# zhuker/lamejs

Measured on AMD Instinct MI355X. Metric: 1152-sample frames/s encoded (44.1kHz 128kbps CBR); bit-exact, higher is better.
Workload: dtype f64; 1 GPU; BASELINE configs[2]: stereo 44.1kHz 128kbps CBR, 1 stream(s) x 100000 synthetic sine frames per GPU; input=Int16 PCM resident in HBM, output=MP3 bytes in HBM, seed_repaired_frames=0, distinct_streams=1, distinct_devices=1

## Files before the change

### lamejs_amd/csrc/k_quant.h

```cpp
#pragma once
#include "lhip_defs.h"
#include "lhip_wave.h"
#include "lhip_math.h"
#include "lhip_layout.h"

namespace lhip {

struct GI {
    double xrpow_max;
    int part2_3_length, big_values, count1, global_gain, scalefac_compress, block_type;
    int table_select[3], subblock_gain[4];
    int region0_count, region1_count, preflag, scalefac_scale, count1table_select;
    int part2_length, sfb_lmax, sfb_smin, psy_lmax, sfbmax, psymax, sfbdivide;
    int count1bits, max_nonzero_coeff;
    int firstcut;
    int tail0;
};

struct NoiseRes { double max_noise; int over_count, over_SSD, bits; };

LHIP_DEV void uni_gi(GI& g) {
    g.xrpow_max = unid(g.xrpow_max);
    g.part2_3_length = uni(g.part2_3_length); g.big_values = uni(g.big_values); g.count1 = uni(g.count1); g.global_gain = uni(g.global_gain);
    g.scalefac_compress = uni(g.scalefac_compress); g.block_type = uni(g.block_type);
    for (int i = 0; i < 3; i++) g.table_select[i] = uni(g.table_select[i]);
    for (int i = 0; i < 4; i++) g.subblock_gain[i] = uni(g.subblock_gain[i]);
    g.region0_count = uni(g.region0_count); g.region1_count = uni(g.region1_count); g.preflag = uni(g.preflag); g.scalefac_scale = uni(g.scalefac_scale);
    g.count1table_select = uni(g.count1table_select); g.part2_length = uni(g.part2_length); g.sfb_lmax = uni(g.sfb_lmax); g.sfb_smin = uni(g.sfb_smin);
    g.psy_lmax = uni(g.psy_lmax); g.sfbmax = uni(g.sfbmax); g.psymax = uni(g.psymax); g.sfbdivide = uni(g.sfbdivide);
    g.count1bits = uni(g.count1bits); g.max_nonzero_coeff = uni(g.max_nonzero_coeff); g.firstcut = uni(g.firstcut); g.tail0 = uni(g.tail0);
}

#if defined(LHIP_PHASE_PROF) && !defined(LHIP_HOSTSIM)
#define PH_BEGIN() const unsigned long long ph_t0_ = __builtin_amdgcn_s_memtime()
#define PH_END(L, id) do { if (lane == 0) { (L).prof[id] += (unsigned int)(__builtin_amdgcn_s_memtime() - ph_t0_); (L).prof[32 + id] += 1; } } while (0)
#define PH_MARK(L, id, t) do { const unsigned long long n_ = __builtin_amdgcn_s_memtime(); if (lane == 0) { (L).prof[id] += (unsigned int)(n_ - (t)); (L).prof[32 + id] += 1; } (t) = n_; } while (0)
#define PH_NOW() __builtin_amdgcn_s_memtime()
#else
#define PH_BEGIN() do {} while (0)
#define PH_END(L, id) do {} while (0)
#define PH_MARK(L, id, t) do {} while (0)
#define PH_NOW() 0ull
#endif
#ifdef LHIP_PROF_BALANCE
#define PH_MARKB(L, id, t) PH_MARK(L, id, t)
#else
#define PH_MARKB(L, id, t) do {} while (0)
#endif
enum { PH_INIT, PH_XRPOW, PH_XMIN, PH_QUANTIZE, PH_COUNT, PH_NOISE, PH_BALANCE, PH_SFSTORE, PH_HUFFDIV, PH_PUBLISH, PH_COPY, PH_TOTAL,
       PH_C_LOAD, PH_C_QUADS, PH_C_MAX, PH_C_SUMS, PH_C_FIN, PH_N_WALK, PH_N_TERMS, PH_N_SUMS, PH_Q_MASK, PH_Q_LINES, PH_N, PH_DRAIN = 29 ,
       PH_N_LINES = 30, PH_N_FOLD = 31 ,
       PH_B_TRIG = 22, PH_B_AMP = 23, PH_B_BREAK = 24, PH_B_BITCOUNT = 25  };

enum { QT_N = 256 };
enum { HL_T1 = 0, HL_T2 = 4, HL_T3 = 13, HL_T5 = 22, HL_T6 = 38, HL_T7 = 54, HL_T8 = 90, HL_T9 = 126, HL_T10 = 162, HL_T11 = 226,
       HL_T12 = 290, HL_T13 = 354, HL_T14 = 610, HL_T15 = 866, HL_EHI = 1122, HL_ELO = 1378, HL_END = 1634 };
LHIP_DEV int hl_off(int t) {
    switch (t) {
        case 1: return HL_T1; case 2: return HL_T2; case 3: return HL_T3; case 5: return HL_T5; case 6: return HL_T6;
        case 7: return HL_T7; case 8: return HL_T8; case 9: return HL_T9; case 10: return HL_T10; case 11: return HL_T11;
        case 12: return HL_T12; case 13: return HL_T13; case 14: return HL_T14; case 15: return HL_T15; default: return 0;
    }
}
struct alignas(16) QuantTabs {
    float pow43[QT_N], adj43[QT_N];
    float ipow20[Q_MAX], pow20[Q_MAX + Q_MAX2 + 1];
    int32_t sfb_l[SBMAX_l + 1], sfb_s[SBMAX_s + 1], pretab[SBMAX_l];
    uint16_t hoff[16];
    uint8_t hlen[HL_END];
    uint8_t t32l[16], t33l[16];
    uint8_t l2s_long[576], l2s_short[576];
    uint32_t bvtab[289];
    uint8_t huf_tbl_noESC[16], ht_xlen[34];
    uint16_t ht_linmax[34];
    struct PlanEnt { uint32_t d0, d1, pw; } plan[30];
    uint32_t sbc[16];
    uint32_t fold_marks[2][64];
    uint16_t wpre_long[24], wpre_short[40];
    int16_t psfb21[PSFB21 + 1], psfb12[PSFB12 + 1];
    float ath_psfb[PSFB21 + PSFB12], fact_psfb[2];
};

LHIP_DEV void q_fill_plans(QuantTabs& Q, int tid, int nthr);

LHIP_DEV void q_load_tabs(const Tables& T, QuantTabs& Q, int tid, int nthr) {
    q_fill_plans(Q, tid, nthr);
    for (int i = tid; i < QT_N; i += nthr) { Q.pow43[i] = T.pow43[i]; Q.adj43[i] = T.adj43[i]; }
    for (int i = tid; i < Q_MAX; i += nthr) Q.ipow20[i] = T.ipow20[i];
    for (int i = tid; i < Q_MAX + Q_MAX2 + 1; i += nthr) Q.pow20[i] = T.pow20[i];
    for (int i = tid; i < 16; i += nthr) { Q.t32l[i] = (uint8_t)T.t32l[i]; Q.t33l[i] = (uint8_t)T.t33l[i]; }
    for (int i = tid; i < SBMAX_l + 1; i += nthr) Q.sfb_l[i] = T.sfb_l[i];
    for (int i = tid; i < SBMAX_s + 1; i += nthr) Q.sfb_s[i] = T.sfb_s[i];
    for (int i = tid; i < SBMAX_l; i += nthr) Q.pretab[i] = T.pretab[i];
    for (int i = tid; i < 16; i += nthr)
        Q.sbc[i] = (uint32_t)T.slen1_n[i] | ((uint32_t)T.slen2_n[i] << 8) | ((uint32_t)T.scale_long[i] << 16) | ((uint32_t)T.scale_short[i] << 24);
    for (int i = tid; i < 289; i += nthr) Q.bvtab[i] = (uint32_t)T.bvtab[i];
    for (int i = tid; i < 15; i += nthr) Q.huf_tbl_noESC[i] = (uint8_t)T.huf_tbl_noESC[i];
    for (int i = tid; i < 34; i += nthr) { Q.ht_xlen[i] = (uint8_t)T.ht_xlen[i]; Q.ht_linmax[i] = (uint16_t)T.ht_linmax[i]; }
    if (tid == 0) { Q.hoff[0] = 0; Q.hoff[4] = 0; }
    for (int t = 1; t < 16; t++) {
        if (t == 4) continue;
        const int xl = T.ht_xlen[t];
        const int n = (t == 14) ? 256 : xl * xl, off = hl_off(t);
        if (tid == 0) Q.hoff[t] = (uint16_t)off;
        for (int i = tid; i < n; i += nthr) Q.hlen[off + i] = (uint8_t)T.ht_hlen[T.ht_off[t] + i];
    }
    for (int i = tid; i < 256; i += nthr) { Q.hlen[HL_EHI + i] = (uint8_t)(T.largetbl[i] >> 16); Q.hlen[HL_ELO + i] = (uint8_t)(T.largetbl[i] & 0xffff); }
    for (int d = tid; d < 576; d += nthr) {
        int sfb = 0;
        while (T.sfb_l[sfb + 1] <= d) sfb++;
        Q.l2s_long[d] = (uint8_t)sfb;
        sfb = 0;
        while (3 * T.sfb_s[sfb + 1] <= d) sfb++;
        const int st = T.sfb_s[sfb], w = T.sfb_s[sfb + 1] - st;
        const int r = d - 3 * st, win = r / w, l = st + (r - win * w);
        Q.l2s_short[d] = (uint8_t)(3 * sfb + win);
        (void)l;
    }
    for (int e = tid; e < PSFB21 + 1; e += nthr) Q.psfb21[e] = (int16_t)T.psfb21[e];
    for (int e = tid; e < PSFB12 + 1; e += nthr) Q.psfb12[e] = (int16_t)T.psfb12[e];
    for (int e = tid; e < PSFB21 + PSFB12; e += nthr) Q.ath_psfb[e] = e < PSFB21 ? T.ATH_psfb21[e] : T.ATH_psfb12[e - PSFB21];
    if (tid == 0) { Q.fact_psfb[0] = T.longfact[21]; Q.fact_psfb[1] = T.shortfact[12]; }
    for (int e = tid; e < 2 * 64; e += nthr) Q.fold_marks[e >> 6][e & 63] = (uint32_t)T.fold_marks[e];
    for (int e = tid; e < 24; e += nthr) Q.wpre_long[e] = (uint16_t)T.wpre[e];
    for (int e = tid; e < 40; e += nthr) Q.wpre_short[e] = (uint16_t)T.wpre[24 + e];
}

LHIP_DEV void q_copy_tabs(const Tables& T, QuantTabs& Q, int tid, int nthr) {
    static_assert(sizeof(QuantTabs) % 16 == 0, "QuantTabs is copied in 16-byte pieces");
    struct alignas(16) V4 { uint32_t a, b, c, d; };
    const V4* src = (const V4*)T.qtabs_img;
    V4* dst = (V4*)&Q;
    for (int i = tid; i < (int)(sizeof(QuantTabs) / 16); i += nthr) dst[i] = src[i];
}

struct QuantLds {
    float xr[576];
    union {
        float xrpow[576];
        struct { int32_t bstat[16][SBMAX_l + 2]; int16_t cand[21][16]; } hd;
    };
    int16_t ixw[576];
    int32_t sfw[SFBMAX + 1], sfb[SFBMAX + 1];
    int16_t width[SFBMAX + 1], window[SFBMAX + 1], start[SFBMAX + 2];
    float xmin[SFBMAX + 1], distort[SFBMAX + 1];
    double rxmin[SFBMAX + 1];
    int32_t pn_step[SFBMAX + 1];
    float pn_dist[SFBMAX + 1];
    union {
        double pn_x[SFBMAX + 1];
        int16_t hmax[5][24];
    };
    int16_t pn_cls[SFBMAX + 1];
    int32_t qmode[SFBMAX + 1];
    float bstep[SFBMAX + 1];
    int8_t sf_gr0[2][SFBMAX + 1];
    union {
        struct { int32_t r01_bits[24], r01_div[24], r0_tbl[24], r1_tbl[24], r2_bits[24], r2_tbl[24]; };
        double nsum[SFBMAX + 1];
        struct { int32_t bs_tab[BS_TAB_MAX], bs_asg[BS_TAB_MAX]; } memo;
    };
    alignas(8) uint32_t rdesc[4][2];
    int32_t gkeep[24];
    double ath_pseudo[PSFB21 + PSFB12];
#ifdef LHIP_PHASE_PROF
    unsigned int prof[64];
#endif
};

LHIP_DEV double ipow20(const QuantTabs& Q, int x) { return (double)Q.ipow20[x]; }
LHIP_DEV double pow20(const QuantTabs& Q, int x) { return (double)Q.pow20[x + Q_MAX2]; }
LHIP_DEV double pow43v(const Tables& T, const QuantTabs& Q, int i) {
    float v = Q.pow43[i < QT_N ? i : QT_N - 1];
    if (i >= QT_N) v = T.pow43[i];
    return (double)v;
}
// ... 702 lines not shown
        if (q.kind == 0) { b = 0; t = 0; }
        if (q.kind == 6) { b = 0; t = 63; }
        PV_(r) = t | ((q.kind == 6) << 6) | (b << 8);
    }
#if LHIP_NL == 1
    const int pv0 = pv[0], pv1_ = pv[1], pv2 = pv[2];
#else
    const int pv0 = wave_bcast(pv1, 0), pv1_ = wave_bcast(pv1, 1), pv2 = wave_bcast(pv1, 2);
#endif
#define APPLY(PV, SLOT) do { const int t_ = (PV) & 63; if ((PV) & 64) bits = LARGE_BITS; else bits += (PV) >> 8; g.table_select[SLOT] = (t_ == 63) ? -1 : t_; } while (0)
    if (use2) APPLY(pv2, 2);
    if (0 < a1) APPLY(pv0, 0);
    if (a1 < a2) APPLY(pv1_, 1);
#undef APPLY
#undef LP_
#undef PV_
    if (use_prev && g.block_type == NORM_TYPE) *pn_sfb_count1 = cnt1_norm;
    PH_MARK(L, PH_C_FIN, tm_);
    return bits;
}

struct PrevNoise { int gain, sfb_count1; };

template <int NR>
LHIP_DEV int q_count_bits(const Tables& T, GI& g, const int32_t* scalefac, int16_t* ix, int use_pn, PrevNoise& pn, int* asg, int lane, QuantLds& L, const QuantTabs& Q) {
    *asg = 0;
    {
        const double ip = ipow20(Q, g.global_gain);
        if (g.xrpow_max * ip > (double)IXMAX_VAL * (1.0 - 0x1p-50)) {
            const double w = (double)IXMAX_VAL / ip;
            if (g.xrpow_max > w) return LARGE_BITS;
        }
    }
    int vx[NR], vy[NR];
    { PH_BEGIN(); q_quantize<NR>(T, g, scalefac, ix, use_pn, use_pn ? pn.gain : 0, use_pn ? pn.sfb_count1 : 0, vx, vy, lane, L, Q); PH_END(L, PH_QUANTIZE); }
    int cnt1 = pn.sfb_count1;
    PH_BEGIN();
    int amask = 0;
    const int r = q_noquant_count_bits<NR>(T, g, ix, vx, vy, use_pn, &cnt1, &amask, lane, L, Q);
    *asg = pack_cond_fields(g, amask);
    if (use_pn) pn.sfb_count1 = cnt1;
    PH_END(L, PH_COUNT);
    return r;
}
template <int SKIP>
LHIP_DEV int q_count_bits_rounds(const Tables& T, GI& g, const int32_t* scalefac, int16_t* ix, int use_pn, PrevNoise& pn, int* asg, int lane, QuantLds& L, const QuantTabs& Q) {
    if constexpr (SKIP != 0) {
        if (g.tail0) { LHIP_ROUND_COUNT(head); return q_count_bits<NPL_HEAD>(T, g, scalefac, ix, use_pn, pn, asg, lane, L, Q); }
    }
    LHIP_ROUND_COUNT(full);
    return q_count_bits<NPL>(T, g, scalefac, ix, use_pn, pn, asg, lane, L, Q);
}

struct NoiseCommit { int fresh, step, cls; float dist; double x; };
LHIP_DEV void q_noise_commit(const GI& g, const NoiseCommit& nc, PrevNoise& pn, int lane, QuantLds& L) {
    lane = fresh_lane(lane);
    LHIP_LANE_ONCE(sfb, 0, g.psymax) {
        if (nc.fresh) { L.pn_step[sfb] = nc.step; L.pn_dist[sfb] = nc.dist; L.pn_x[sfb] = nc.x; L.pn_cls[sfb] = (int16_t)nc.cls; }
    }
    pn.gain = g.global_gain;
    wave_sync();
}
LHIP_DEV void q_calc_noise_(const Tables& T, const GI& g, const int32_t* scalefac, const int16_t* ix, NoiseRes* res,
                           int use_pn, PrevNoise& pn, int need_max, int lane, QuantLds& L, const QuantTabs& Q, NoiseCommit* defer = nullptr) {
    lane = fresh_lane(lane);
    unsigned long long tm_ = PH_NOW(); (void)tm_;
    const int is_short = g.block_type == SHORT_TYPE;
    const int may_big = !(g.xrpow_max * ipow20(Q, g.global_gain) < (double)(QT_N - 1));
#if LHIP_NL == 1
    const uint8_t* l2s = line2sfb(Q, g.block_type);
    int over = 0, ssd = 0;
    uint64_t m_fresh = 0;
    (void)may_big; (void)is_short;
    for (int sfb = 0; sfb < g.psymax; sfb++) {
        const int s = sf_step(Q, g, scalefac, L.window, sfb);
        if (!(use_pn && L.pn_step[sfb] == s)) m_fresh |= 1ull << sfb;
        L.qmode[sfb] = s;
        L.bstep[sfb] = Q.pow20[s + Q_MAX2];
    }
    PH_MARK(L, PH_N_WALK, tm_);
    {
        double sacc = 0.0;
        for (int j = 0; j < 576; j++) {
            const int bnd = l2s[j];
            if (j == 0 || l2s[j - 1] != bnd) sacc = 0.0;
            const double x = __builtin_fma(-pow43v(T, Q, ix[j]), (double)L.bstep[bnd < SFBMAX + 1 ? bnd : SFBMAX], d_abs((double)L.xr[j]));
            sacc += x * x;
            if (j == 575 || l2s[j + 1] != bnd) L.nsum[bnd] = sacc;
        }
    }
    PH_MARK(L, PH_N_FOLD, tm_);
    for (int sfb = 0; sfb < g.psymax; sfb++) {
        int cls;
        if (!((m_fresh >> sfb) & 1)) { L.distort[sfb] = L.pn_dist[sfb]; cls = L.pn_cls[sfb]; }
        else {
            const double noise = L.nsum[sfb], b = (double)L.xmin[sfb], rb = L.rxmin[sfb];
            const double x = rb != 0.0 ? div_by_f32(noise, b, rb) : noise / b;
            L.distort[sfb] = (float)x;
            if (use_pn) { L.pn_step[sfb] = L.qmode[sfb]; const double nf = (double)(float)noise; L.pn_dist[sfb] = (float)(rb != 0.0 ? div_by_f32(nf, b, rb) : nf / b); }
            cls = need_max ? -1 : noise_class(x);
            int cls_cache = cls;
            if (cls < 0) {
                const double l = v8_log10_pos(x > 1E-20 ? x : 1E-20);
                cls = noise_class_of_log(l); cls_cache = noise_class_of_log((double)(float)l);
            }
            if (use_pn) { L.pn_x[sfb] = x; L.pn_cls[sfb] = (int16_t)cls_cache; }
            else L.nsum[sfb] = x;
        }
        if (cls > 0) { ssd += cls * cls; over++; }
    }
    PH_MARK(L, PH_N_TERMS, tm_);
    if (use_pn) pn.gain = g.global_gain;
    res->over_count = over; res->over_SSD = ssd;
    res->max_noise = 0.0;
    if (need_max || over == 0) {
        double max_noise = -20.0;
        for (int sfb = 0; sfb < g.psymax; sfb++) {
            const bool fresh = (m_fresh >> sfb) & 1;
            const double x = (fresh && !use_pn) ? L.nsum[sfb] : L.pn_x[sfb];
            const double l = v8_log10_pos(x > 1E-20 ? x : 1E-20);
            const double nl = fresh ? l : (double)(float)l;
            if (nl > max_noise) max_noise = nl;
        }
        res->max_noise = max_noise;
    }
#else
    int my_step = 0, my_fresh = 0;
    LHIP_LANE_ONCE(sfb, 0, g.psymax) {
        my_step = sf_step(Q, g, scalefac, L.window, sfb);
        my_fresh = !(use_pn && L.pn_step[sfb] == my_step);
        L.bstep[sfb] = Q.pow20[my_step + Q_MAX2];
    }
    const uint64_t m_fresh = wave_ballot(my_fresh);
    const int hib = m_fresh ? 63 - (int)__builtin_clzll(m_fresh) : 0;
    const int maxlen = m_fresh ? (int)(is_short ? Q.wpre_short[hib] : Q.wpre_long[hib]) : 0;
    wave_sync();
    PH_MARK(L, PH_N_WALK, tm_);
    enum { NLN = 576 / LHIP_NL };
    static_assert(NLN == 9, "QuantTabs::fold_marks is laid out for 9 lines per lane");
    {
        double tq[NLN], keep[NLN];
        int lastb[NLN];
        const uint32_t marks = Q.fold_marks[is_short][lane];
        const uint8_t* l2s = line2sfb(Q, g.block_type);
#define NOISE_TERMS(IDX) _Pragma("unroll") for (int k = 0; k < NLN; k++) { \
            const int j = NLN * lane + k; \
            const int bnd = l2s[j]; \
            const float bstep = L.bstep[bnd]; \
            const float xa = L.xr[j]; const int iv = ix[j]; \
            const float pw = Q.pow43[IDX]; \
            const double x = __builtin_fma(-(double)pw, (double)bstep, d_abs((double)xa)); \
            tq[k] = x * x; \
            keep[k] = one_unless_bit(marks, k); \
            lastb[k] = bnd; \
        }
        if (!may_big) { NOISE_TERMS(iv) } else { NOISE_TERMS(iv < QT_N ? iv : QT_N - 1) }
#undef NOISE_TERMS
        if (may_big) {
#pragma unroll
            for (int k = 0; k < NLN; k++) {
                const int j = NLN * lane + k;
                const int iv = ix[j];
                if (iv >= QT_N) {
                    const double x = __builtin_fma(-(double)T.pow43[iv], (double)L.bstep[lastb[k]], d_abs((double)L.xr[j]));
                    tq[k] = x * x;
                }
            }
        }
        PH_MARK(L, PH_N_LINES, tm_);
        const int nsteps = (maxlen + NLN - 1) / NLN + 1;
        double carry = 0.0;
        for (int st = 0; st + 1 < nsteps; st++) {
            double sacc = carry;
#pragma unroll
            for (int k = 0; k < NLN; k++) sacc = __builtin_fma(sacc, keep[k], tq[k]);
            carry = wave_shr1d(sacc, 0.0);
        }
        {
            double sacc = carry;
#pragma unroll
            for (int k = 0; k < NLN; k++) { sacc = __builtin_fma(sacc, keep[k], tq[k]); tq[k] = sacc; }
        }
#pragma unroll
        for (int k = 0; k < NLN; k++) if ((marks >> (16 + k)) & 1u) L.nsum[lastb[k]] = tq[k];
        wave_sync();
        PH_MARK(L, PH_N_FOLD, tm_);
    }
    double x = 1.0;
    int cls = 0;
    const int fresh = my_fresh;
    LHIP_LANE_ONCE(sfb, 0, g.psymax) {
        if (!fresh) {
            L.distort[sfb] = L.pn_dist[sfb];
            x = L.pn_x[sfb];
            cls = L.pn_cls[sfb];
        } else {
            const double noise = L.nsum[sfb], b = (double)L.xmin[sfb], rb = L.rxmin[sfb];
            const double nf = (double)(float)noise;
            x = div_by_f32(noise, b, rb);
            double xf = div_by_f32(nf, b, rb);
            if (rb == 0.0) { x = noise / b; xf = nf / b; }
            L.distort[sfb] = (float)x;
            if (defer) { defer->step = my_step; defer->dist = (float)xf; }
            else if (use_pn) { L.pn_step[sfb] = my_step; L.pn_dist[sfb] = (float)xf; }
            cls = need_max ? -1 : noise_class(x);
        }
    }
    PH_MARK(L, PH_N_TERMS, tm_);
    int cls_cache = cls;
    int have_log = 0;
    double nl = -20.0;
    if (wave_any(cls < 0)) {
        LHIP_LANE_ONCE(sfb, 0, g.psymax) {
            const double l = v8_log10_pos(x > 1E-20 ? x : 1E-20);
            const double lf = (double)(float)l;
            nl = fresh ? l : lf;
            if (fresh) { cls = noise_class_of_log(l); cls_cache = noise_class_of_log(lf); }
        }
        have_log = 1;
    }
    int over = 0, ssd = 0;
    if (defer) { defer->fresh = 0; LHIP_LANE_ONCE(sfb, 0, g.psymax) { defer->fresh = use_pn && fresh; defer->x = x; defer->cls = cls_cache; } }
    LHIP_LANE_ONCE(sfb, 0, g.psymax) {
        if (!defer && use_pn && fresh) { L.pn_x[sfb] = x; L.pn_cls[sfb] = (int16_t)cls_cache; }
        if (cls > 0) { ssd = cls * cls; over = 1; }
    }
    if (use_pn && !defer) pn.gain = g.global_gain;
    {
        const int os = wave_sum((ssd << 6) | over);
        res->over_count = os & 63; res->over_SSD = os >> 6;
    }
    res->max_noise = 0.0;
    if (need_max || res->over_count == 0) {
        double max_noise = -20.0;
        if (!have_log) {
            LHIP_LANE_ONCE(sfb, 0, g.psymax) {
                const double l = v8_log10_pos(x > 1E-20 ? x : 1E-20);
                nl = fresh ? l : (double)(float)l;
            }
        }
// ... 1496 lines not shown
```

### lamejs_amd/csrc/lhip_api.cpp

```cpp
#include "../../include/lamejs_hip.h"
#include "lhip_defs.h"
#include "lhip_wave.h"
#include "lhip_math.h"
#include "lhip_layout.h"
#include "k_psy.h"
#include "k_fb.h"
#include "k_quant.h"
#if !defined(LHIP_HOSTSIM) || defined(LHIP_WAVESIM)
#include "k_quant_tail.h"
#endif
#include "k_quant_fast.h"
#include "k_bits.h"
#include "k_crc.h"
#include "k_ingest.h"
#include "k_gain.h"

#include <string>
#include <vector>
#include <map>
#include <mutex>
#include <thread>
#include <atomic>
#include <memory>
#include <cstring>
// ... 564 lines not shown
    (void)device;
#endif
    return 0;
}

int lhip_set_hip_stream(int device, void* hip_stream) {
#ifndef LHIP_HOSTSIM
    if (device < 0) { if (hipGetDevice(&device) != hipSuccess) return LHIP_ERR_INTERNAL; }
#else
    if (device < 0) device = 0;
#endif
    Context* ctx = get_context(device);
    std::lock_guard<std::mutex> lk(ctx->mu);
    ctx->stream = hip_stream;
    return 0;
}

void lhip_last_batch_stats(int64_t* frames, int64_t* repaired_frames, int64_t* repair_iterations) {
#ifndef LHIP_HOSTSIM
    if (g_stat_pending) {
        Context* ctx = g_stat_pending;
        g_stat_pending = nullptr;
        std::lock_guard<std::mutex> lk(ctx->mu);
        int32_t fx[3] = {0, 0, 0};
        WorkSet& ws = ctx->ws;
        void* st = ctx->stream;
        if (rt::set_device(ctx->device) && rt::d2h(fx, (const int32_t*)ws.nflagged.p + FX_STATS, sizeof fx, st) && rt::sync(st)) {
            g_stat_repaired = fx[0]; g_stat_iters = fx[1];
            if (fx[2]) set_err("seed-chain repair did not converge");
        }
    }
#endif
    if (frames) *frames = g_stat_frames;
    if (repaired_frames) *repaired_frames = g_stat_repaired;
    if (repair_iterations) *repair_iterations = g_stat_iters;
}

int lhip_debug_last_paths(uint32_t* mask) {
    if (!mask) { set_err("lhip_debug_last_paths: null argument"); return LHIP_ERR_INTERNAL; }
    *mask = g_last_paths;
    return 0;
}

int64_t lhip_debug_read(int what, void* dst, size_t cap) {
    if (what == 11) {
        if (!dst) { set_err("lhip_debug_read: null argument"); return LHIP_ERR_INTERNAL; }
        const size_t n = cap < sizeof g_last_quant ? cap : sizeof g_last_quant; memcpy(dst, &g_last_quant, n); return (int64_t)n;
    }
#ifdef LHIP_HOSTSIM
    if (what == 10) {
        const int64_t v[2] = {(int64_t)__atomic_load_n(&round_stats().head, __ATOMIC_RELAXED), (int64_t)__atomic_load_n(&round_stats().full, __ATOMIC_RELAXED)};
        const size_t n = cap < sizeof v ? cap : sizeof v; memcpy(dst, v, n); return (int64_t)n;
    }
#endif
#ifdef LHIP_PHASE_PROF
    if (what == 9) { const size_t n = cap < sizeof g_call_prof ? cap : sizeof g_call_prof; memcpy(dst, g_call_prof, n); return (int64_t)n; }
#endif
    Context* ctx = nullptr;
    { std::lock_guard<std::mutex> lk(g_ctx_mu); for (auto& kv : g_ctx) if (kv.second->ws.have_last) ctx = kv.second.get(); }
    if (!ctx) { set_err("no batch has run"); return LHIP_ERR_INTERNAL; }
    std::lock_guard<std::mutex> lk(ctx->mu);
    rt::set_device(ctx->device);
    const WorkSet& ws = ctx->ws;
    const Workspace& W = ws.lastW;
    const size_t GC = (size_t)W.ngslots * ws.lastC;
    const void* src = nullptr; size_t n = 0;
    switch (what) {
        case 0: src = W.xr; n = GC * 576 * 4; break;
        case 1: src = W.blocktype; n = GC * 4; break;
        case 2: src = W.E; n = (size_t)W.ngslots * ws.lastCp * E_STRIDE * 4; break;
        case 3: src = W.ath_adjust; n = (size_t)W.nfslots * 8; break;
        case 4: src = W.side; n = (size_t)W.nframes_total * 2 * ws.lastC * sizeof(GrSide); break;
        case 5: src = W.sb; n = GC * SB_STRIDE * 4; break;
        case 6: src = W.peaks; n = GC * PK_STRIDE * 4; break;
        case 7: src = W.prof; n = PROF_BYTES; break;
        case 8: src = W.nflagged; n = 256; break;
        default: set_err("unknown tap"); return LHIP_ERR_INTERNAL;
    }
    if (n > cap) n = cap;
    if (!rt::d2h(dst, src, n, ctx->stream) || !rt::sync(ctx->stream)) return LHIP_ERR_INTERNAL;
    return (int64_t)n;
}

int lhip_stream_info(const lhip_stream* s, lhip_stream_info_t* info) {
    if (!s || s->magic != 0x4c484950) { set_err("bad stream handle"); return LHIP_ERR_BAD_HANDLE; }
    if (!info) { set_err("lhip_stream_info: null argument"); return LHIP_ERR_INTERNAL; }
    if (!s->tag) { set_err("lhip_stream_info: the stream was not created with the infoTag option (its totals are not kept)"); return LHIP_ERR_INTERNAL; }
    const TagTotals& v = *s->tag;
    info->frames = v.frames; info->audio_bytes = v.bytes; info->music_crc = v.crc & 0xffff; info->delay = s->ts->tag.delay;
    info->padding = v.padding < 0 ? -1 : (int32_t)v.padding; info->tag_bytes = s->ts->tag.size;
    return 0;
}
int64_t lhip_info_tag(lhip_stream* s, uint8_t* out, size_t cap) {
    if (!s || s->magic != 0x4c484950) { set_err("bad stream handle"); return LHIP_ERR_BAD_HANDLE; }
    if (!s->tag) { set_err("lhip_info_tag: the stream was not created with the infoTag option"); return LHIP_ERR_INTERNAL; }
    if (s->tag->moved) { set_err("lhip_info_tag: the stream was moved with lhip_seek or lhip_state_set; state blobs do not carry the tag's totals (combining the tags of shards is not supported)"); return LHIP_ERR_INTERNAL; }
    if (!s->tag->flushed) { set_err("lhip_info_tag: the stream has not been flushed (the tag reports the totals and the end padding of the complete stream)"); return LHIP_ERR_INTERNAL; }
    const size_t n = (size_t)s->ts->tag.size;
    if (!out || cap < n) { set_err("output buffer too small"); return LHIP_ERR_BUFFER_TOO_SMALL; }
    uint32_t radio = 0;
    if (s->gain) {
        int32_t tenth = 0; int64_t windows = 0, samples = 0;
        const int rc = lhip_replay_gain(s, &tenth, &windows, &samples);
        if (rc < 0) return rc;
        if (rc == 0) radio = gain_tag_field(tenth);
    }
// ... 234 lines not shown
```

### lamejs_amd/csrc/lhip_defs.h

```cpp
#pragma once
#include <stdint.h>
#include <stddef.h>

#ifdef LHIP_HOSTSIM
#include <math.h>
#include <string.h>
#include <stdio.h>
#include <stdlib.h>
#define LHIP_DEV static inline
#ifdef LHIP_WAVESIM
#define LHIP_NL 64
#else
#define LHIP_NL 1
#endif
#else
#include <hip/hip_runtime.h>
#define LHIP_DEV static __device__ __forceinline__
#define LHIP_NL 64
#endif

#ifdef LHIP_HOSTSIM
typedef const double* lhip_ctab;
#define LHIP_CTAB(p) (p)
#define LHIP_SCHED_FENCE() ((void)0)
// ... 15 lines not shown

namespace lhip {

enum {
    SBMAX_l = 22, SBMAX_s = 13, SBPSY_l = 21, SBPSY_s = 12, PSFB21 = 6, PSFB12 = 6,
    CBANDS = 64, BLKSIZE = 1024, HBLKSIZE = 513, BLKSIZE_s = 256, HBLKSIZE_s = 129, SFBMAX = 39,
    NORM_TYPE = 0, START_TYPE = 1, SHORT_TYPE = 2, STOP_TYPE = 3,
    IXMAX_VAL = 8206, PRECALC_SIZE = IXMAX_VAL + 2, Q_MAX = 257, Q_MAX2 = 116, LARGE_BITS = 100000,
    MAX_BITS_PER_CHANNEL = 4095, MAX_BITS_PER_GRANULE = 7680,
    FRAME = 1152, GRAN = 576, MF_NEEDED = 1904, MF_INIT = 528
};

#define LHIP_SQRT2 1.41421356237309504880

struct Tables {
    int channels_out, mode, mode_gr, version, samplerate_index, bitrate_index, brate, out_samplerate,
        sideinfo_len, frac_SpF, noise_shaping, noise_shaping_amp, noise_shaping_stop, subblock_gain,
        use_best_huffman, full_outer_loop, substep_shaping, sfb21_extra, quant_comp, quant_comp_short,
        short_blocks_coupled, useTemporal, ATH_useAdjust, athaa_loudapprox, copyright, original, emphasis,
        extension, error_protection, npart_l, npart_s, n_version_bytes,
        n_s3_ll,
       
        in_samplerate, rs_filter_l, rs_bpc,
        rs_ratio,
        rs_frac,
        psy_channels,
        disable_reservoir;
    double scale, attackthre, attackthre_s, interChRatio, masking_lower_long, masking_lower_short,
        ATH_aaSensitivityP, ATH_floor, decay, ma_max_i1, ma_max_i2, ma_max_m, VO_SCALE, resample_ratio,
        msfix, ATHlower;
    const float *rs_blackfilt;
    const float *amp_filter, *ATH_l, *ATH_s, *ATH_psfb21, *ATH_psfb12, *ATH_cb_l, *ATH_cb_s, *eql_w,
        *pow43, *adj43, *ipow20, *pow20, *longfact, *shortfact, *rnumlines_l, *bo_l_weight, *bo_s_weight,
        *s3_ll, *s3_ss, *window, *window_s, *mld_l, *mld_s;
    const int32_t *sfb_l, *sfb_s, *psfb21, *psfb12, *bv_scf, *numlines_l, *numlines_s, *bo_l, *bm_l, *bo_s,
        *bm_s, *s3ind, *s3ind_s, *fft_rv_tbl, *mdct_order, *pretab, *scfsi_band, *slen1_n, *slen2_n,
        *slen1_tab, *slen2_tab, *scale_short, *scale_long, *huf_tbl_noESC, *version_bytes, *ht_xlen,
        *ht_linmax, *ht_off, *ht_code, *ht_hlen, *largetbl, *table23, *table56, *t32l, *t33l;
    const double *fht_twiddle, *fht_costab, *enwindow, *mdct_win, *ma_tab, *ma_table1, *ma_table2, *ma_table3,
        *hpf_fircoef;
    const int32_t *s3off_l, *s3off_s;
    const int32_t *lineoff_l, *lineoff_s;
    const double *amp_by_out;
    int amp_mask;
    const int32_t *psy_fold; int psy_maxlen_l;
    const int32_t *bvtab;
    const void *qtabs_img;
    const int32_t *fold_marks, *wpre;
    double scale_left, scale_right;
    int channels_in,
        do_scale, do_scale_left, do_scale_right,
        in_mix;
    float pcm_limit;
};

enum { BS_TAB_MAX = 24 };
struct GrSide {
    int32_t part2_3_length, part2_length, big_values, count1, global_gain, scalefac_compress, block_type;
    int32_t table_select[3], subblock_gain[3];
    int32_t region0_count, region1_count, preflag, scalefac_scale, count1table_select;
    int32_t sfbmax, sfbdivide;
    int32_t active;
    int32_t bs_start, bs_step_in, bs_gain;
    int32_t targ_bits;
    int32_t scfsi;
    int32_t scalefac[SFBMAX];
    int32_t bs_ntab, bs_tab[BS_TAB_MAX];
    int32_t bs_asg[BS_TAB_MAX], bs_state;
    int32_t mode_ext;
};

}
```

### lamejs_amd/csrc/lhip_kernels.h

```cpp
#pragma once
#define XCD_GRID(n) (8 * (((n) + 7) / 8))
static __device__ __forceinline__ int xcd_item(int b, int n) { const int it = (b & 7) * ((n + 7) >> 3) + (b >> 3); return it < n && (b >> 3) < ((n + 7) >> 3) ? it : -1; }
__global__ __launch_bounds__(64) void g_load(Tables T, Workspace W, const StreamDesc* SD, const StreamIO* IO) { kb_load(T, W, SD, IO, blockIdx.x, threadIdx.x); }
__global__ __launch_bounds__(64) void g_save(Tables T, Workspace W, const StreamDesc* SD, const StreamIO* IO) { kb_save(T, W, SD, IO, blockIdx.x, threadIdx.x); }
#ifndef LHIP_WPB
#define LHIP_WPB 4
#endif
enum { WPB = LHIP_WPB };
#define XCD_GRID_W(n) XCD_GRID(((n) + WPB - 1) / WPB)
static __device__ __forceinline__ int xcd_wave_item(int n, int* lane) {
    const int wv = __builtin_amdgcn_readfirstlane((int)(threadIdx.x >> 6));
    *lane = (int)(threadIdx.x & 63);
    const int g = xcd_item(blockIdx.x, (n + WPB - 1) / WPB);
    const int it = g * WPB + wv;
    return (g >= 0 && it < n) ? it : -1;
}
#define WAVE_LDS(TYPE, NAME) __shared__ TYPE NAME##_[WPB]; TYPE& NAME = NAME##_[__builtin_amdgcn_readfirstlane((int)(threadIdx.x >> 6))]
__global__ __launch_bounds__(64 * WPB) void g_psyA(Tables T, Workspace W, const StreamDesc* SD, const StreamIO* IO, int chn0, int nch) {
    WAVE_LDS(PsyALds, L);
    int lane;
    const int it = xcd_wave_item(W.ngslots * nch, &lane);
    if (it >= 0) kb_psyA(T, W, SD, IO, it / nch, chn0 + it % nch, lane, L);
}
__global__ __launch_bounds__(256) void g_prep(Tables T, Workspace W, const StreamDesc* SD, const StreamIO* IO, int nstreams) {
// ... 46 lines not shown
    __shared__ QuantTabs Q;
    __shared__ QuantLds L[QWAVES];
    __shared__ TailShare TS;
#ifndef LHIP_PHASE_PROF
    static_assert(QWAVES * sizeof(QuantLds) + sizeof(QuantTabs) + sizeof(TailShare) <= 80 * 1024, "g_quant: LDS budget for 2 workgroups per CU exceeded");
#endif
    const QArgs* A = (const QArgs*)__builtin_amdgcn_kernarg_segment_ptr();
    q_copy_tabs(A->T, Q, threadIdx.x, 64 * QWAVES);
    if (threadIdx.x == 0) TS.drawing = QWAVES;
    if (threadIdx.x < QWAVES) TS.offer[threadIdx.x].state = 0;
    const bool tail_help_on = !RESV && A->T.channels_out == 2;
    __syncthreads();
    const int wv = __builtin_amdgcn_readfirstlane(threadIdx.x >> 6);
#ifdef LHIP_PHASE_PROF
    L[wv].prof[threadIdx.x & 63] = 0;
#endif
#if defined(LHIP_PHASE_PROF) || defined(LHIP_WAVE_TIMES)
    const unsigned long long wave_t0_ = wall_clock64();
#endif
    int hint[3] = {-1, -1, -1};
    for (;;) {
        const int fslot = next_frame_slot(A->W.work_ctr + A->ctr);
        if (fslot >= A->nfs) break;
        if constexpr (!RESV) kb_quant_th<SKIP>(A->T, A->pb, A->W, A->SD, fslot, threadIdx.x & 63, L[wv], Q, hint, TS, wv);
        else kb_quant<0, RESV, SKIP>(A->T, A->pb, A->W, A->SD, fslot, A->chain, threadIdx.x & 63, L[wv], Q, -1, nullptr, nullptr, nullptr);
        hint[0] = __builtin_amdgcn_readfirstlane(hint[0]); hint[1] = __builtin_amdgcn_readfirstlane(hint[1]); hint[2] = __builtin_amdgcn_readfirstlane(hint[2]);
    }
    if (tail_help_on) tail_help<SKIP>(A->T, A->pb, A->W, A->SD, threadIdx.x & 63, L, wv, QWAVES, Q, TS);
#ifdef LHIP_PHASE_PROF
    atomicAdd((unsigned long long*)A->W.prof + (threadIdx.x & 63), (unsigned long long)L[wv].prof[threadIdx.x & 63]);
#endif
#if defined(LHIP_PHASE_PROF) || defined(LHIP_WAVE_TIMES)
    {
        const int wid = blockIdx.x * QWAVES + wv;
        if ((threadIdx.x & 63) == 0 && wid < 8192) { A->W.prof[64 + 2 * wid] = wave_t0_; A->W.prof[64 + 2 * wid + 1] = wall_clock64(); }
    }
#endif
}
template <int RESV, int SKIP> __global__ __launch_bounds__(128, LHIP_QOCC) void g_quant_pair(QArgs a_unused) {
    __shared__ QuantTabs Q;
    __shared__ QuantLds L[2];
    __shared__ int mbox[4];
    const QArgs* A = (const QArgs*)__builtin_amdgcn_kernarg_segment_ptr();
    q_copy_tabs(A->T, Q, threadIdx.x, 128);
    __syncthreads();
    const int wv = __builtin_amdgcn_readfirstlane(threadIdx.x >> 6);
    kb_quant<1, RESV, SKIP>(A->T, A->pb, A->W, A->SD, blockIdx.x, A->chain, threadIdx.x & 63, L[wv], Q, wv, mbox);
}
enum { QF_WAVES = 8 };
template <int PAIR, int SKIP> __global__ __launch_bounds__(64 * QF_WAVES, LHIP_QOCC) void g_quant_fast(QArgs a_unused) {
    __shared__ QuantTabs Q;
    __shared__ QuantLds L[QF_WAVES];
    __shared__ FastPair FP[QF_WAVES / 2];
    static_assert(QF_WAVES * sizeof(QuantLds) + sizeof(QuantTabs) + sizeof(FP) <= 80 * 1024, "g_quant_fast: LDS budget for 2 workgroups per CU exceeded");
    static_assert(sizeof(FP) / sizeof(int) <= 64 * QF_WAVES, "the pair records are zeroed by one store per thread");
    const QArgs* A = (const QArgs*)__builtin_amdgcn_kernarg_segment_ptr();
    q_copy_tabs(A->T, Q, threadIdx.x, 64 * QF_WAVES);
    if (threadIdx.x < sizeof(FP) / sizeof(int)) ((int*)FP)[threadIdx.x] = 0;
    __syncthreads();
    const int wv = __builtin_amdgcn_readfirstlane(threadIdx.x >> 6), lane = threadIdx.x & 63;
    int hint[3] = {-1, -1, -1};
    for (int round = 1;; round++) {
        int fslot;
        if constexpr (PAIR != 0) {
            FastPair& fp = FP[wv >> 1];
            if ((wv & 1) == 0) { fslot = next_frame_slot(A->W.work_ctr + A->ctr); fast_pair_publish_slot(fp, round, fslot, lane); }
            else fslot = fast_pair_await_slot(fp, round, lane);
            if (fslot >= A->nfs) break;
            kb_quant_fast<1, SKIP>(A->T, A->pb, A->W, A->SD, fslot, lane, L[wv], Q, hint, wv & 1, &fp, round);
        } else {
            fslot = next_frame_slot(A->W.work_ctr + A->ctr);
            if (fslot >= A->nfs) break;
            kb_quant_fast<0, SKIP>(A->T, A->pb, A->W, A->SD, fslot, lane, L[wv], Q, hint);
        }
        hint[0] = __builtin_amdgcn_readfirstlane(hint[0]); hint[1] = __builtin_amdgcn_readfirstlane(hint[1]); hint[2] = __builtin_amdgcn_readfirstlane(hint[2]);
    }
}
__global__ __launch_bounds__(256) void g_validate_fast(Tables T, Workspace W, const StreamDesc* SD, int nfs) {
    __shared__ ValidateShare S;
    const int t = blockIdx.x * 256 + threadIdx.x, fslot = t >> 2;
    kb_validate_fast_quad(T, W, SD, fslot < nfs ? fslot : 0, t & 3, fslot < nfs, S);
}
enum { FX_NFLAG = 0, FX_NSLOW = 1, FX_WORK_REPAIR = 2, FX_WORK_SLOW = 3, FX_PARITY_STRIDE = 8, FX_BAR = 24, FX_STATS = 32 };
LHIP_DEV void grid_barrier(int32_t* bar, int nblocks) {
    __syncthreads();
    if (nblocks > 1 && threadIdx.x == 0) {
        __builtin_amdgcn_fence(__ATOMIC_RELEASE, "agent");
        asm volatile("s_waitcnt vmcnt(0)" ::: "memory");
        const int gen = __hip_atomic_load(bar + 1, __ATOMIC_RELAXED, __HIP_MEMORY_SCOPE_AGENT);
        if (__hip_atomic_fetch_add(bar, 1, __ATOMIC_RELAXED, __HIP_MEMORY_SCOPE_AGENT) == nblocks - 1) {
            __hip_atomic_store(bar, 0, __ATOMIC_RELAXED, __HIP_MEMORY_SCOPE_AGENT);
            __builtin_amdgcn_fence(__ATOMIC_RELEASE, "agent");
            asm volatile("s_waitcnt vmcnt(0)" ::: "memory");
            __hip_atomic_fetch_add(bar + 1, 1, __ATOMIC_RELAXED, __HIP_MEMORY_SCOPE_AGENT);
        } else {
            for (int n = 0; __hip_atomic_load(bar + 1, __ATOMIC_RELAXED, __HIP_MEMORY_SCOPE_AGENT) == gen; n++) { if (n > (1 << 26)) __builtin_trap(); __builtin_amdgcn_s_sleep(4); }
        }
        __builtin_amdgcn_fence(__ATOMIC_ACQUIRE, "agent");
    }
    __syncthreads();
}
#ifndef LHIP_FIXUP_OCC
#define LHIP_FIXUP_OCC 4
#endif
template <int SKIP> __global__ __launch_bounds__(64 * QWAVES, LHIP_FIXUP_OCC) void g_fixup(QArgs a_unused) {
    __shared__ QuantTabs Q;
    __shared__ QuantLds L[QWAVES];
// ... 187 lines not shown
```

### lamejs_amd/csrc/lhip_tables.h

```cpp
#pragma once
struct lhtb_entry { char name[32]; uint32_t dtype, count, offset, pad; };

struct TableSet {
    Tables T;
    PowBase pb10;
    std::vector<uint8_t> blob;
    void* d_blob = nullptr;
    void* d_extra = nullptr;
    void* d_qtabs = nullptr;
    int device = 0;
    int base_frame_bytes = 0;
    bool bad_option = false;
    InfoTagCfg tag;
    bool skip_tail = false;
    int gain_on = 0;
    bool fast = false;
    ~TableSet() { rt::dfree(d_blob); rt::dfree(d_extra); rt::dfree(d_qtabs); }
};

static bool fast_quant_allowed() { static const bool off = []() { const char* e = getenv("LAMEJS_HIP_NO_FAST_QUANT"); return e && e[0] == '1'; }(); return !off; }

static const lhtb_entry* find_entry(const uint8_t* b, const char* name) {
    uint32_t n; memcpy(&n, b + 8, 4);
    const lhtb_entry* e = (const lhtb_entry*)(b + 16);
// ... 173 lines not shown
    std::vector<int32_t> extra(4 * CBANDS, 0);
    int k = 0, j = 0;
    for (int p = 0; p < T.npart_l; p++) { extra[p] = k; k += h_s3ind[2 * p + 1] - h_s3ind[2 * p] + 1; extra[2 * CBANDS + p] = j; j += h_nl[p]; }
    if (j != HBLKSIZE) { set_err("long partitions do not cover 513 lines"); return false; }
    T.n_s3_ll = k;
    if (k > PSYB_S3_LDS) { set_err("configuration outside the supported envelope (spreading table larger than g_psyB's LDS copy)"); return false; }
    k = 0; j = 0;
    for (int p = 0; p < T.npart_s; p++) { extra[CBANDS + p] = k; k += h_s3ind_s[2 * p + 1] - h_s3ind_s[2 * p] + 1; extra[3 * CBANDS + p] = j; j += h_ns[p]; }
    if (j != HBLKSIZE_s) { set_err("short partitions do not cover 129 lines"); return false; }
    auto walk = [&](const int32_t* bo, int nb, int npart, int32_t* stop) {
        int b = 0, sb = 0;
        for (; sb < nb; ++b, ++sb) {
            const int lim = bo[sb] < npart ? bo[sb] : npart;
            if (b < lim) b = lim;
            stop[sb] = b;
            if (b >= npart) { ++sb; break; }
        }
        for (; sb < nb; ++sb) stop[sb] = npart;
    };
    extra.resize(4 * CBANDS + SBMAX_l + SBMAX_s);
    walk(h_bo_l, SBMAX_l, T.npart_l, extra.data() + 4 * CBANDS);
    walk(h_bo_s, SBMAX_s, T.npart_s, extra.data() + 4 * CBANDS + SBMAX_l);
    const size_t amp_at = (extra.size() + 1) & ~(size_t)1;
    extra.resize(amp_at + 64);
    {
        const float* h_af = (const float*)host_arr("amp_filter");
        for (int band = 0; band < 32; band++)
            if (!std::isfinite(h_af[band]) || h_af[band] < 0.f || h_af[band] > 1.f) { set_err("band filter: amp_filter[" + std::to_string(band) + "] is not a finite value in [0, 1]"); ts.bad_option = true; return false; }
        ts.skip_tail = (double)h_af[28] < 1e-12 && (double)h_af[29] < 1e-12 && (double)h_af[30] < 1e-12 && (double)h_af[31] < 1e-12;
        const int32_t* h_order = (const int32_t*)host_arr("mdct_order");
        double amp[32];
        for (int i = 0; i < 32; i++) amp[i] = 1.0;
        T.amp_mask = 0;
        for (int band = 0; band < 32; band++) {
            const double af = (double)h_af[band];
            const int ob = h_order[band];
            if (ob < 0 || ob > 31) { set_err("mdct_order is not a permutation of 0..31"); return false; }
            if (!(af < 1e-12) && af < 1.0) { amp[ob] = af; T.amp_mask |= 1 << ob; }
        }
        memcpy(extra.data() + amp_at, amp, sizeof amp);
    }
    const size_t fold_at = extra.size();
    extra.resize(fold_at + 128 + 24 + 40 + 289);
    {
        const int32_t* h_sl = (const int32_t*)host_arr("sfb_l");
        const int32_t* h_ss = (const int32_t*)host_arr("sfb_s");
        std::vector<int> band_l(576), band_s(576);
        for (int d = 0, sfb = 0; d < 576; d++) { while (sfb < SBMAX_l - 1 && h_sl[sfb + 1] <= d) sfb++; band_l[d] = sfb; }
        for (int d = 0, sfb = 0; d < 576; d++) {
            while (sfb < SBMAX_s - 1 && 3 * h_ss[sfb + 1] <= d) sfb++;
            const int st = h_ss[sfb], w = h_ss[sfb + 1] - st;
            band_s[d] = 3 * sfb + (w > 0 ? (d - 3 * st) / w : 0);
        }
        for (int sh = 0; sh < 2; sh++) {
            const std::vector<int>& b = sh ? band_s : band_l;
            for (int ln = 0; ln < 64; ln++) {
                uint32_t m = 0;
                for (int kk = 0; kk < 9; kk++) {
                    const int jj = 9 * ln + kk;
                    if (jj == 0 || b[jj - 1] != b[jj]) m |= 1u << kk;
                    if (jj == 575 || b[jj + 1] != b[jj]) m |= 1u << (16 + kk);
                }
                extra[fold_at + 64 * sh + ln] = (int32_t)m;
            }
        }
        int mx = 0;
        for (int i = 0; i < 24; i++) { if (i < SBMAX_l) { const int w = h_sl[i + 1] - h_sl[i]; if (mx < w) mx = w; } extra[fold_at + 128 + i] = mx; }
        mx = 0;
        for (int i = 0; i < 40; i++) { if (i < 3 * SBMAX_s) { const int w = h_ss[i / 3 + 1] - h_ss[i / 3]; if (mx < w) mx = w; } extra[fold_at + 128 + 24 + i] = mx; }
        {
            const int32_t* h_bv = (const int32_t*)host_arr("bv_scf");
            extra[fold_at + 128 + 24 + 40] = 0;
            for (int e = 1; e <= 288; e++) {
                const int i = 2 * e, r0 = h_bv[i - 2], r1 = h_bv[i - 1];
                if (r0 < 0 || r0 > 15 || r1 < 0 || r1 > 7 || r0 + r1 + 2 > SBMAX_l) { set_err("bv_scf outside the range count_bits' region table is packed for"); return false; }
                const int a1 = h_sl[r0 + 1], a2 = h_sl[r0 + r1 + 2];
                extra[fold_at + 128 + 24 + 40 + e] = (int32_t)((uint32_t)a1 | ((uint32_t)a2 << 10) | ((uint32_t)r0 << 20) | ((uint32_t)r1 << 24) | ((uint32_t)(band_l[i - 1] + 1) << 27));
            }
        }
    }
    const size_t psyfold_at = extra.size();
    extra.resize(psyfold_at + 3 * 64);
    {
        std::vector<int> part(514, 0);
        for (int p = 0, jj = 0; p < T.npart_l; p++) for (int i = 0; i < h_nl[p] && jj < 513; i++) part[jj++] = p;
        part[513] = -1;
        int mx = 0;
        for (int p = 0; p < T.npart_l; p++) if (mx < h_nl[p]) mx = h_nl[p];
        T.psy_maxlen_l = mx;
        for (int ln = 0; ln < 64; ln++) {
            uint32_t m = 0, w[2] = {0, 0};
            for (int kk = 0; kk < 8; kk++) {
                const int jj = 8 * ln + kk;
                if (jj == 0 || part[jj - 1] != part[jj]) m |= 1u << kk;
                if (part[jj + 1] != part[jj]) m |= 1u << (8 + kk);
                w[kk >> 2] |= (uint32_t)part[jj] << (8 * (kk & 3));
            }
            extra[psyfold_at + 3 * ln] = (int32_t)m; extra[psyfold_at + 3 * ln + 1] = (int32_t)w[0]; extra[psyfold_at + 3 * ln + 2] = (int32_t)w[1];
        }
        const float* h_eql = (const float*)host_arr("eql_w");
        for (int i = 0; i < BLKSIZE / 2; i++) if (!(h_eql[i] >= 0.f)) { set_err("eql_w has a negative entry (the loudness sum's error bound needs non-negative terms)"); return false; }
    }
    ts.d_extra = rt::dmalloc(extra.size() * 4);
    if (!ts.d_extra) { set_err("hipMalloc failed"); return false; }
    if (!rt::h2d(ts.d_extra, extra.data(), extra.size() * 4, stream)) return false;
    if (!rt::sync(stream)) return false;
    T.s3off_l = (const int32_t*)ts.d_extra; T.s3off_s = T.s3off_l + CBANDS; T.lineoff_l = T.s3off_l + 2 * CBANDS; T.lineoff_s = T.s3off_l + 3 * CBANDS;
    T.bo_l = T.s3off_l + 4 * CBANDS; T.bo_s = T.bo_l + SBMAX_l;
    T.amp_by_out = (const double*)(T.s3off_l + amp_at);
    T.fold_marks = T.s3off_l + fold_at; T.wpre = T.fold_marks + 128; T.bvtab = T.wpre + 64;
    T.psy_fold = T.s3off_l + psyfold_at;
    return true;
}
static bool build_tables(TableSet& ts, const void* blob, size_t nbytes, const lhip_config& cfg, void* stream) {
    if (!parse_blob(ts, blob, nbytes, stream) || !check_envelope(ts, cfg) || !derive_index_tables(ts, stream)) return false;
    Tables& T = ts.T;
    ts.d_qtabs = rt::dmalloc(sizeof(QuantTabs));
// ... 18 lines not shown
```

Before: 2.349 million frames/s.

## Narrow per-lane noise line count when only low bands or psy range need folding

Turns the per-lane noise band summation into a template over lines per lane (3, 7 or 9). A 3-line variant covering the first 192 lines runs when all fresh bands lie in that region, and a 7-line variant runs when the psychoacoustic band limit fits in 448 lines. Both skip distortion terms for lines that cannot contribute. Host-built fold-mark masks now also hold 3-line boundary bits, and a host-sim counter records which variant ran. Risks are code-size growth, more register pressure from three instantiations, and a possible bit-exactness change if the skipped lines mattered.

Result: faster. 2.389 million frames/s, median of 6 (+1.7%).

```diff
diff --git a/lamejs_amd/csrc/k_quant.h b/lamejs_amd/csrc/k_quant.h
--- a/lamejs_amd/csrc/k_quant.h
+++ b/lamejs_amd/csrc/k_quant.h
@@ -76,6 +76,7 @@
     struct PlanEnt { uint32_t d0, d1, pw; } plan[30];
     uint32_t sbc[16];
     uint32_t fold_marks[2][64];
+    int32_t noise_nln;
     uint16_t wpre_long[24], wpre_short[40];
     int16_t psfb21[PSFB21 + 1], psfb12[PSFB12 + 1];
     float ath_psfb[PSFB21 + PSFB12], fact_psfb[2];
@@ -122,6 +123,7 @@
     for (int e = tid; e < PSFB21 + PSFB12; e += nthr) Q.ath_psfb[e] = e < PSFB21 ? T.ATH_psfb21[e] : T.ATH_psfb12[e - PSFB21];
     if (tid == 0) { Q.fact_psfb[0] = T.longfact[21]; Q.fact_psfb[1] = T.shortfact[12]; }
     for (int e = tid; e < 2 * 64; e += nthr) Q.fold_marks[e >> 6][e & 63] = (uint32_t)T.fold_marks[e];
+    if (tid == 0) Q.noise_nln = T.noise_nln;
     for (int e = tid; e < 24; e += nthr) Q.wpre_long[e] = (uint16_t)T.wpre[e];
     for (int e = tid; e < 40; e += nthr) Q.wpre_short[e] = (uint16_t)T.wpre[24 + e];
 }
@@ -930,6 +932,69 @@
     return q_count_bits<NPL>(T, g, scalefac, ix, use_pn, pn, asg, lane, L, Q);
 }
 
+#if defined(LHIP_HOSTSIM)
+struct NoiseLineStats { long n7 = 0, n9 = 0, n3 = 0; };
+inline NoiseLineStats& noise_line_stats() { static NoiseLineStats t; return t; }
+#define LHIP_NOISE_LINES_COUNT(f) do { if (lane == 0) __atomic_fetch_add(&noise_line_stats().f, 1L, __ATOMIC_RELAXED); } while (0)
+#else
+#define LHIP_NOISE_LINES_COUNT(f) do { } while (0)
+#endif
+#if LHIP_NL != 1
+template <int NLN>
+LHIP_DEV void q_noise_band_sums(const Tables& T, const GI& g, const int16_t* ix, int may_big, int maxlen, int lane, QuantLds& L, const QuantTabs& Q,
+                                unsigned long long& tm_) {
+    static_assert(LHIP_NL == 64 && (NLN == 3 || NLN == 7 || NLN == 9), "QuantTabs::fold_marks is laid out for 3 and for 7 or 9 lines on each of 64 lanes");
+    enum { MS = NLN == 3 ? 12 : 0 };
+    if (NLN == 3) LHIP_NOISE_LINES_COUNT(n3); else if (NLN == 7) LHIP_NOISE_LINES_COUNT(n7); else LHIP_NOISE_LINES_COUNT(n9);
+    double tq[NLN], keep[NLN];
+    int lastb[NLN];
+    const uint32_t marks = Q.fold_marks[g.block_type == SHORT_TYPE][lane];
+    const uint8_t* l2s = line2sfb(Q, g.block_type);
+#define NOISE_TERMS(IDX) _Pragma("unroll") for (int k = 0; k < NLN; k++) { \
+        const int j = NLN * lane + k; \
+        const int bnd = l2s[j]; \
+        const float bstep = L.bstep[bnd]; \
+        const float xa = L.xr[j]; const int iv = ix[j]; \
+        const float pw = Q.pow43[IDX]; \
+        const double x = __builtin_fma(-(double)pw, (double)bstep, d_abs((double)xa)); \
+        tq[k] = x * x; \
+        keep[k] = one_unless_bit(marks, MS + k); \
+        lastb[k] = bnd; \
+    }
+    if (!may_big) { NOISE_TERMS(iv) } else { NOISE_TERMS(iv < QT_N ? iv : QT_N - 1) }
+#undef NOISE_TERMS
+    if (may_big) {
+#pragma unroll
+        for (int k = 0; k < NLN; k++) {
+            const int j = NLN * lane + k;
+            const int iv = ix[j];
+            if (iv >= QT_N) {
+                const double x = __builtin_fma(-(double)T.pow43[iv], (double)L.bstep[lastb[k]], d_abs((double)L.xr[j]));
+                tq[k] = x * x;
+            }
+        }
+    }
+    PH_MARK(L, PH_N_LINES, tm_);
+    const int nsteps = (maxlen + NLN - 1) / NLN + 1;
+    double carry = 0.0;
+    for (int st = 0; st + 1 < nsteps; st++) {
+        double sacc = carry;
+#pragma unroll
+        for (int k = 0; k < NLN; k++) sacc = __builtin_fma(sacc, keep[k], tq[k]);
+        carry = wave_shr1d(sacc, 0.0);
+    }
+    {
+        double sacc = carry;
+#pragma unroll
+        for (int k = 0; k < NLN; k++) { sacc = __builtin_fma(sacc, keep[k], tq[k]); tq[k] = sacc; }
+    }
+#pragma unroll
+    for (int k = 0; k < NLN; k++) if ((marks >> (16 + MS + k)) & 1u) L.nsum[lastb[k]] = tq[k];
+    wave_sync();
+    PH_MARK(L, PH_N_FOLD, tm_);
+}
+#endif
+
 struct NoiseCommit { int fresh, step, cls; float dist; double x; };
 LHIP_DEV void q_noise_commit(const GI& g, const NoiseCommit& nc, PrevNoise& pn, int lane, QuantLds& L) {
     lane = fresh_lane(lane);
@@ -1014,56 +1079,9 @@
     const int maxlen = m_fresh ? (int)(is_short ? Q.wpre_short[hib] : Q.wpre_long[hib]) : 0;
     wave_sync();
     PH_MARK(L, PH_N_WALK, tm_);
-    enum { NLN = 576 / LHIP_NL };
-    static_assert(NLN == 9, "QuantTabs::fold_marks is laid out for 9 lines per lane");
-    {
-        double tq[NLN], keep[NLN];
-        int lastb[NLN];
-        const uint32_t marks = Q.fold_marks[is_short][lane];
-        const uint8_t* l2s = line2sfb(Q, g.block_type);
-#define NOISE_TERMS(IDX) _Pragma("unroll") for (int k = 0; k < NLN; k++) { \
-            const int j = NLN * lane + k; \
-            const int bnd = l2s[j]; \
-            const float bstep = L.bstep[bnd]; \
-            const float xa = L.xr[j]; const int iv = ix[j]; \
-            const float pw = Q.pow43[IDX]; \
-            const double x = __builtin_fma(-(double)pw, (double)bstep, d_abs((double)xa)); \
-            tq[k] = x * x; \
-            keep[k] = one_unless_bit(marks, k); \
-            lastb[k] = bnd; \
-        }
-        if (!may_big) { NOISE_TERMS(iv) } else { NOISE_TERMS(iv < QT_N ? iv : QT_N - 1) }
-#undef NOISE_TERMS
-        if (may_big) {
-#pragma unroll
-            for (int k = 0; k < NLN; k++) {
-                const int j = NLN * lane + k;
-                const int iv = ix[j];
-                if (iv >= QT_N) {
-                    const double x = __builtin_fma(-(double)T.pow43[iv], (double)L.bstep[lastb[k]], d_abs((double)L.xr[j]));
-                    tq[k] = x * x;
-                }
-            }
-        }
-        PH_MARK(L, PH_N_LINES, tm_);
-        const int nsteps = (maxlen + NLN - 1) / NLN + 1;
-        double carry = 0.0;
-        for (int st = 0; st + 1 < nsteps; st++) {
-            double sacc = carry;
-#pragma unroll
-            for (int k = 0; k < NLN; k++) sacc = __builtin_fma(sacc, keep[k], tq[k]);
-            carry = wave_shr1d(sacc, 0.0);
-        }
-        {
-            double sacc = carry;
-#pragma unroll
-            for (int k = 0; k < NLN; k++) { sacc = __builtin_fma(sacc, keep[k], tq[k]); tq[k] = sacc; }
-        }
-#pragma unroll
-        for (int k = 0; k < NLN; k++) if ((marks >> (16 + k)) & 1u) L.nsum[lastb[k]] = tq[k];
-        wave_sync();
-        PH_MARK(L, PH_N_FOLD, tm_);
-    }
+    if (m_fresh && hib <= T.noise_hib3[is_short]) q_noise_band_sums<3>(T, g, ix, may_big, maxlen, lane, L, Q, tm_);
+    else if (T.noise_nln == 7) q_noise_band_sums<7>(T, g, ix, may_big, maxlen, lane, L, Q, tm_);
+    else q_noise_band_sums<9>(T, g, ix, may_big, maxlen, lane, L, Q, tm_);
     double x = 1.0;
     int cls = 0;
     const int fresh = my_fresh;
diff --git a/lamejs_amd/csrc/lhip_api.cpp b/lamejs_amd/csrc/lhip_api.cpp
--- a/lamejs_amd/csrc/lhip_api.cpp
+++ b/lamejs_amd/csrc/lhip_api.cpp
@@ -640,6 +640,10 @@
         const int64_t v[2] = {(int64_t)__atomic_load_n(&round_stats().head, __ATOMIC_RELAXED), (int64_t)__atomic_load_n(&round_stats().full, __ATOMIC_RELAXED)};
         const size_t n = cap < sizeof v ? cap : sizeof v; memcpy(dst, v, n); return (int64_t)n;
     }
+    if (what == 12) {
+        const int64_t v[3] = {(int64_t)__atomic_load_n(&noise_line_stats().n7, __ATOMIC_RELAXED), (int64_t)__atomic_load_n(&noise_line_stats().n9, __ATOMIC_RELAXED), (int64_t)__atomic_load_n(&noise_line_stats().n3, __ATOMIC_RELAXED)};
+        const size_t n = cap < sizeof v ? cap : sizeof v; memcpy(dst, v, n); return (int64_t)n;
+    }
 #endif
 #ifdef LHIP_PHASE_PROF
     if (what == 9) { const size_t n = cap < sizeof g_call_prof ? cap : sizeof g_call_prof; memcpy(dst, g_call_prof, n); return (int64_t)n; }
diff --git a/lamejs_amd/csrc/lhip_defs.h b/lamejs_amd/csrc/lhip_defs.h
--- a/lamejs_amd/csrc/lhip_defs.h
+++ b/lamejs_amd/csrc/lhip_defs.h
@@ -91,6 +91,8 @@
         do_scale, do_scale_left, do_scale_right,
         in_mix;
     float pcm_limit;
+    int noise_nln;
+    int noise_hib3[2];
 };
 
 enum { BS_TAB_MAX = 24 };
diff --git a/lamejs_amd/csrc/lhip_kernels.h b/lamejs_amd/csrc/lhip_kernels.h
--- a/lamejs_amd/csrc/lhip_kernels.h
+++ b/lamejs_amd/csrc/lhip_kernels.h
@@ -122,7 +122,9 @@
     __shared__ QuantTabs Q;
     __shared__ QuantLds L[QF_WAVES];
     __shared__ FastPair FP[QF_WAVES / 2];
+#ifndef LHIP_PHASE_PROF
     static_assert(QF_WAVES * sizeof(QuantLds) + sizeof(QuantTabs) + sizeof(FP) <= 80 * 1024, "g_quant_fast: LDS budget for 2 workgroups per CU exceeded");
+#endif
     static_assert(sizeof(FP) / sizeof(int) <= 64 * QF_WAVES, "the pair records are zeroed by one store per thread");
     const QArgs* A = (const QArgs*)__builtin_amdgcn_kernarg_segment_ptr();
     q_copy_tabs(A->T, Q, threadIdx.x, 64 * QF_WAVES);
diff --git a/lamejs_amd/csrc/lhip_tables.h b/lamejs_amd/csrc/lhip_tables.h
--- a/lamejs_amd/csrc/lhip_tables.h
+++ b/lamejs_amd/csrc/lhip_tables.h
@@ -249,17 +249,27 @@
             const int st = h_ss[sfb], w = h_ss[sfb + 1] - st;
             band_s[d] = 3 * sfb + (w > 0 ? (d - 3 * st) / w : 0);
         }
+        const int nln = (h_sl[SBPSY_l] <= 64 * 7 && 3 * h_ss[SBPSY_s] <= 64 * 7) ? 7 : 9;
+        T.noise_nln = nln;
         for (int sh = 0; sh < 2; sh++) {
             const std::vector<int>& b = sh ? band_s : band_l;
             for (int ln = 0; ln < 64; ln++) {
                 uint32_t m = 0;
-                for (int kk = 0; kk < 9; kk++) {
-                    const int jj = 9 * ln + kk;
+                for (int kk = 0; kk < nln; kk++) {
+                    const int jj = nln * ln + kk;
                     if (jj == 0 || b[jj - 1] != b[jj]) m |= 1u << kk;
                     if (jj == 575 || b[jj + 1] != b[jj]) m |= 1u << (16 + kk);
                 }
+                for (int kk = 0; kk < 3; kk++) {
+                    const int jj = 3 * ln + kk;
+                    if (jj == 0 || b[jj - 1] != b[jj]) m |= 1u << (12 + kk);
+                    if (b[jj + 1] != b[jj]) m |= 1u << (28 + kk);
+                }
                 extra[fold_at + 64 * sh + ln] = (int32_t)m;
             }
+            int hb = -1;
+            for (int jj = 0; jj < 192; jj++) if (b[jj + 1] != b[jj]) hb = b[jj];
+            T.noise_hib3[sh] = hb;
         }
         int mx = 0;
         for (int i = 0; i < 24; i++) { if (i < SBMAX_l) { const int w = h_sl[i + 1] - h_sl[i]; if (mx < w) mx = w; } extra[fold_at + 128 + i] = mx; }
```
